# zju3dv/pvnet

Hardware: NVIDIA H100
Metric: images/sec (480x640, K=9) backbone+vote (higher is better)
Workload: dtype tf32 (fp32 storage, fp32 accumulate; vote fp32/fp64)

## Files before the change

pvnet_b200/csrc/conv_col.cu:

```cuda
#include "conv_tc.cuh"
#include "ptx.cuh"

#include <cstdlib>
#include <mutex>
#include <new>

namespace pvnet {

int g_conv_mode = 0;

namespace {

constexpr int COL_TH = 16, COL_TW = 8;
constexpr int COL_THREADS = 384;
constexpr int HEAD_MAX = 64;

__host__ __device__ constexpr int head_pitch(int hc) { return hc <= 8 ? 8 : (hc <= 24 ? 24 : 40); }
constexpr int HEAD_CPITCH = COL_TH * COL_TW + 4;
__host__ __device__ constexpr int head_stage_floats(int hc)
{
    return COL_TH * COL_TW * head_pitch(hc) > hc * HEAD_CPITCH ? COL_TH * COL_TW * head_pitch(hc) : hc * HEAD_CPITCH;
}
__host__ __device__ constexpr int head_stage_bytes(int hc) { return (head_stage_floats(hc) * 4 + COL_TH * COL_TW + 127) & ~127; }

struct ColGeom {
    int Ho, Wo, tiles_x, tiles_y, total_tiles;
    int cin_chunks, cin_pad;
    int split_chunk;
    int pad_l, pad_t;
    int stages;
    int resident;
    int out_cs, out_co, res_cs, res_co;
    int act, round_out;
    int head_cout, head_seg, mask_esz;
    int head_nhwc;
};

__device__ __forceinline__ void head_store_tile(const ColGeom &g, uint32_t sv, uint32_t sm, float *head_out, void *mask,
                                                int img, int y0, int x0, int tid, int nthr)
{
    const int hc = g.head_cout, pp = head_pitch(hc);
    const int nx = min(COL_TW, g.Wo - x0), ny = min(COL_TH, g.Ho - y0);
    const size_t npix = (size_t)g.Ho * g.Wo;
    const bool vec = (reinterpret_cast<uintptr_t>(head_out) & 15) == 0 && (g.head_nhwc ? hc % 4 == 0 : g.Wo % 4 == 0);
    for (int u = tid; u < 32 * hc; u += nthr) {
        if (g.head_nhwc) {
            const int r = u / (2 * hc), e0 = 4 * (u - r * 2 * hc);
            if (r >= ny) continue;
            float *dst = head_out + (((size_t)img * g.Ho + y0 + r) * g.Wo + x0) * hc + e0;
            if (vec) {
                const int col = e0 / hc;
                if (col < nx)
                    *reinterpret_cast<float4 *>(dst) = ptx::lds128(sv + 4u * (uint32_t)((r * COL_TW + col) * pp + e0 - col * hc));
            } else {
#pragma unroll
                for (int i = 0; i < 4; ++i) {
                    const int col = (e0 + i) / hc;
                    if (col < nx) dst[i] = ptx::lds32(sv + 4u * (uint32_t)((r * COL_TW + col) * pp + e0 + i - col * hc));
                }
            }
        } else {
            const int co = u >> 5, r = (u >> 1) & 15, xo = 4 * (u & 1);
            if (r >= ny) continue;
            float *dst = head_out + ((size_t)img * hc + co) * npix + (size_t)(y0 + r) * g.Wo + x0 + xo;
            const uint32_t src = sv + 4u * (uint32_t)(co * HEAD_CPITCH + r * COL_TW + xo);
            if (vec) {
                if (xo < nx) *reinterpret_cast<float4 *>(dst) = ptx::lds128(src);
            } else {
#pragma unroll
                for (int i = 0; i < 4; ++i)
                    if (xo + i < nx) dst[i] = ptx::lds32(src + 4u * i);
            }
        }
    }
    if (!mask) return;
    for (int p = tid; p < COL_TH * COL_TW; p += nthr) {
        const int r = p / COL_TW, c = p % COL_TW;
        if (r >= ny || c >= nx) continue;
        const size_t pix = ((size_t)img * g.Ho + y0 + r) * g.Wo + x0 + c;
        const uint32_t v = ptx::lds8(sm + (uint32_t)p);
        if (g.mask_esz == 8) reinterpret_cast<long long *>(mask)[pix] = v;
        else reinterpret_cast<unsigned char *>(mask)[pix] = (unsigned char)v;
    }
}

template <int KC, bool HEAD, int KH, int BN, bool WIDE = false>
__global__ void __launch_bounds__(COL_THREADS, 1)
    k_conv_col(const __grid_constant__ CUtensorMap tmA, const __grid_constant__ CUtensorMap tmA2,
               const __grid_constant__ CUtensorMap tmB, const __grid_constant__ CUtensorMap tmBw, const __grid_constant__ ColGeom g,
               const float *__restrict__ bias, const float *__restrict__ res, float *__restrict__ out,
               const float *__restrict__ head_w, const float *__restrict__ head_b, float *__restrict__ head_out,
               void *__restrict__ mask)
{
    static_assert(!HEAD || BN == 32, "fused head: 32 input channels");
    static_assert(!HEAD || KC == 8, "fused head: convraw.0's 8-channel chunks");
    static_assert((KC == 16) == (KH == 4), "16-channel chunks are the 4x4 stem's, and only its");
    static_assert(!WIDE || (HEAD && KC == 8 && KH == 3), "wide first source: convraw.0 form only");
    constexpr int ROWB = KC * 4;
    constexpr int B_TILE = BN * ROWB;
    constexpr int PITCH = COL_TW + KH - 1;
    constexpr int A_BOX = (COL_TH + KH - 1) * PITCH * ROWB;
    constexpr int A_BYTES = (A_BOX + 1023) & ~1023;
    constexpr int WIDE_BOX = (COL_TH + KH - 1) * PITCH * 128;
    constexpr int WIDE_BYTES = (WIDE_BOX + 1023) & ~1023;
    extern __shared__ uint8_t smem_raw[];
    uint8_t *smem = reinterpret_cast<uint8_t *>((reinterpret_cast<uintptr_t>(smem_raw) + 1023) & ~uintptr_t(1023));
    const int n_btiles = KH * KH * g.cin_chunks;
    const int n_loads = WIDE ? 2 : g.cin_chunks;
    const int stage_bytes = WIDE ? WIDE_BYTES : A_BYTES + (g.resident ? 0 : KH * KH * B_TILE);
    uint8_t *sB = smem;
    uint8_t *sA = smem + (g.resident ? (size_t)n_btiles * B_TILE : 0);
    uint8_t *sH = sA + (size_t)g.stages * stage_bytes;
    uint8_t *sHS = sH + (HEAD ? 4096 : 0);
    const int hs_bytes = HEAD ? head_stage_bytes(g.head_cout) : 0;
    uint64_t *wfull = reinterpret_cast<uint64_t *>(sHS + 2 * hs_bytes);
    uint64_t *full = wfull + 1;
    uint64_t *empty = full + g.stages;
    uint64_t *hstaged = empty + g.stages;
    uint64_t *hfree = hstaged + 2;
    float *s_bias = reinterpret_cast<float *>(empty + g.stages + (HEAD ? 4 : 0));
    float *s_head = s_bias + 64;
    constexpr int STORE_THREADS = 96;

    const int warp = threadIdx.x >> 5, lane = threadIdx.x & 31;
    if (threadIdx.x == 0) {
        ptx::mbar_init(wfull, 1);
        for (int s = 0; s < g.stages; ++s) {
            ptx::mbar_init(&full[s], 1);
            ptx::mbar_init(&empty[s], 8);
        }
        if (HEAD)
            for (int b = 0; b < 2; ++b) {
                ptx::mbar_init(&hstaged[b], 256);
                ptx::mbar_init(&hfree[b], STORE_THREADS);
            }
        ptx::fence_barrier_init();
    }
    for (int i = threadIdx.x; i < BN; i += blockDim.x) s_bias[i] = bias[i];
    if (HEAD) {
        for (int i = threadIdx.x; i < 32; i += blockDim.x) s_head[i] = i < g.head_cout ? head_b[i] : 0.f;
        for (int i = threadIdx.x; i < 32 * 32; i += blockDim.x) {
            const int n = i >> 5, p = i & 31, q = p & 7;
            const int k = (p & ~7) + (q < 4 ? 2 * q : 2 * (q - 4) + 1);
            const float v = n < g.head_cout ? head_w[n * 32 + k] : 0.f;
            *reinterpret_cast<float *>(sH + ptx::swizzle_off((uint32_t)(n * 128 + p * 4), 128)) = v;
        }
        ptx::fence_proxy_async();
    }
    __syncthreads();
    const int tiles_per_img = g.tiles_x * g.tiles_y;

    if (warp >= 8) {
        const int pw = warp - 8;
        if (pw == 0 && lane == 0 && g.resident) {
            ptx::mbar_arrive_expect_tx(wfull, (uint32_t)(n_btiles * B_TILE));
            for (int cc = WIDE ? g.split_chunk : 0; cc < g.cin_chunks; ++cc)
                for (int t = 0; t < KH * KH; ++t)
                    ptx::tma_load_2d(sB + (size_t)(cc * KH * KH + t) * B_TILE, &tmB, wfull, t * g.cin_pad + cc * KC, 0);
            if (WIDE)
                for (int t = 0; t < KH * KH; ++t) ptx::tma_load_2d(sB + (size_t)t * BN * 128, &tmBw, wfull, t * g.cin_pad, 0);
        }
        if (HEAD && pw != 0) {
            const int tid = threadIdx.x - 9 * 32;
            int it = 0;
            for (int tile = blockIdx.x; tile < g.total_tiles; tile += gridDim.x, ++it) {
                const int b = it & 1;
                const int img = tile / tiles_per_img;
                const int trem = tile - img * tiles_per_img;
                const int tyi = trem / g.tiles_x, txi = trem - tyi * g.tiles_x;
                const uint32_t buf = ptx::smem_u32(sHS) + (uint32_t)(b * hs_bytes);
                ptx::mbar_wait(&hstaged[b], (uint32_t)(it >> 1) & 1u);
                head_store_tile(g, buf, buf + 4u * (uint32_t)head_stage_floats(g.head_cout), head_out, mask, img, tyi * COL_TH,
                                txi * COL_TW, tid, STORE_THREADS);
                ptx::mbar_arrive(&hfree[b]);
            }
            return;
        }
        if (pw != 0) return;
        int s = 0;
        uint32_t ph = 0;
        const uint32_t tx_bytes = (uint32_t)(A_BOX + (g.resident ? 0 : KH * KH * B_TILE));
        for (int tile = blockIdx.x; tile < g.total_tiles; tile += gridDim.x) {
            const int img = tile / tiles_per_img;
            const int trem = tile - img * tiles_per_img;
            const int tyi = trem / g.tiles_x, txi = trem - tyi * g.tiles_x;
            const int y0 = tyi * COL_TH, x0 = txi * COL_TW;
            for (int cc = 0; cc < n_loads; ++cc) {
                uint8_t *st = sA + (size_t)s * stage_bytes;
                if (WIDE) {
                    if (pw == 0 && lane == 0) {
                        ptx::mbar_wait(&empty[s], ph ^ 1u);
                        ptx::mbar_arrive_expect_tx(&full[s], (uint32_t)(cc == 0 ? WIDE_BOX : A_BOX));
                        ptx::tma_load_4d(st, cc == 0 ? &tmA : &tmA2, &full[s], 0, x0 - g.pad_l, y0 - g.pad_t, img);
                    }
                    __syncwarp();
                } else if (pw == 0) {
                    if (lane == 0) {
                        ptx::mbar_wait(&empty[s], ph ^ 1u);
                        ptx::mbar_arrive_expect_tx(&full[s], tx_bytes);
                        if (cc < g.split_chunk)
                            ptx::tma_load_4d(st, &tmA, &full[s], cc * KC, x0 - g.pad_l, y0 - g.pad_t, img);
                        else
                            ptx::tma_load_4d(st, &tmA2, &full[s], (cc - g.split_chunk) * KC, x0 - g.pad_l, y0 - g.pad_t, img);
                        if (!g.resident)
                            for (int t = 0; t < KH * KH; ++t)
                                ptx::tma_load_2d(st + A_BYTES + (size_t)t * B_TILE, &tmB, &full[s], t * g.cin_pad + cc * KC, 0);
                    }
                    __syncwarp();
                }
                if (++s == g.stages) {
                    s = 0;
                    ph ^= 1u;
                }
            }
        }
        return;
    }

    const int wg = warp >> 2, wq = warp & 3;
    const int g8 = lane >> 2, t4 = lane & 3;
    const uint32_t sA_u = ptx::smem_u32(sA), sB_u = ptx::smem_u32(sB);
    if (g.resident) ptx::mbar_wait(wfull, 0);
    int s = 0;
    uint32_t ph = 0;
    int it = 0;
    for (int tile = blockIdx.x; tile < g.total_tiles; tile += gridDim.x, ++it) {
        float acc[BN / 2];
#pragma unroll
        for (int i = 0; i < BN / 2; ++i) acc[i] = 0.f;
        int prev = -1;
        for (int cc = 0; cc < n_loads; ++cc) {
            ptx::mbar_wait(&full[s], ph);
            const uint32_t a0 = sA_u + (uint32_t)s * (uint32_t)stage_bytes;
            ptx::wgmma_fence();
            if (WIDE && cc == 0) {
                const uint64_t ad0 = ptx::make_kmajor_desc(a0 + (uint32_t)(8 * wg * PITCH * 128), 128, PITCH * 128);
                const uint64_t bd0 = ptx::make_kmajor_desc(sB_u, 128);
#pragma unroll
                for (int ks = 0; ks < 4; ++ks)
#pragma unroll
                    for (int t = 0; t < KH * KH; ++t)
                        ptx::Wgmma<BN>::ss(acc, ad0 + (uint64_t)(((t / KH) * PITCH + t % KH) * 128 / 16 + 2 * ks),
                                           bd0 + (uint64_t)(t * (BN * 128) / 16 + 2 * ks), (t | ks) != 0 ? 1u : 0u);
            } else {
                const int c8 = WIDE ? g.split_chunk : cc;
                const uint32_t b0 = g.resident ? sB_u + (uint32_t)(c8 * KH * KH * B_TILE) : a0 + (uint32_t)A_BYTES;
                const uint64_t ad0 = ptx::make_kmajor_desc(a0 + (uint32_t)(8 * wg * PITCH * ROWB), ROWB, PITCH * ROWB);
                const uint64_t bd0 = ptx::make_kmajor_desc(b0, ROWB);
#pragma unroll
                for (int t = 0; t < KH * KH; ++t) {
                    const uint64_t ad = ad0 + (uint64_t)(((t / KH) * PITCH + t % KH) * ROWB / 16);
                    const uint64_t bd = bd0 + (uint64_t)(t * B_TILE / 16);
#pragma unroll
                    for (int ks = 0; ks < KC / 8; ++ks)
                        ptx::Wgmma<BN>::ss(acc, ad + (uint64_t)(2 * ks), bd + (uint64_t)(2 * ks), (c8 | t | ks) != 0 ? 1u : 0u);
                }
            }
            ptx::wgmma_commit();
            ptx::wgmma_wait<1>();
            ptx::fence_regs(acc);
            if (prev >= 0 && lane == 0) ptx::mbar_arrive(&empty[prev]);
            prev = s;
            if (++s == g.stages) {
                s = 0;
                ph ^= 1u;
            }
        }
        ptx::wgmma_wait<0>();
        ptx::fence_regs(acc);
        if (lane == 0) ptx::mbar_arrive(&empty[prev]);

        const int img = tile / tiles_per_img;
        const int trem = tile - img * tiles_per_img;
        const int tyi = trem / g.tiles_x, txi = trem - tyi * g.tiles_x;
        const int ty = 8 * wg + 2 * wq;
        if constexpr (!HEAD) {
            bool ok[2];
            size_t pix[2];
#pragma unroll
            for (int h = 0; h < 2; ++h) {
                const int y = tyi * COL_TH + ty + h, x = txi * COL_TW + g8;
                ok[h] = y < g.Ho && x < g.Wo;
                pix[h] = ok[h] ? ((size_t)img * g.Ho + y) * g.Wo + x : 0;
            }
            float2 rv[2][BN / 8];
            if (res) {
#pragma unroll
                for (int h = 0; h < 2; ++h)
#pragma unroll
                    for (int j = 0; j < BN / 8; ++j)
                        rv[h][j] = ok[h] ? __ldg(reinterpret_cast<const float2 *>(res + pix[h] * g.res_cs + g.res_co + 8 * j + 2 * t4))
                                         : make_float2(0.f, 0.f);
            }
#pragma unroll
            for (int h = 0; h < 2; ++h) {
                if (!ok[h]) continue;
                float *optr = out + pix[h] * g.out_cs + g.out_co;
#pragma unroll
                for (int j = 0; j < BN / 8; ++j) {
                    const int c = 8 * j + 2 * t4;
                    float2 v = make_float2(acc[4 * j + 2 * h] + s_bias[c], acc[4 * j + 2 * h + 1] + s_bias[c + 1]);
                    if (res) {
                        v.x += rv[h][j].x;
                        v.y += rv[h][j].y;
                    }
                    v.x = epi_act(v.x, g.act, g.round_out);
                    v.y = epi_act(v.y, g.act, g.round_out);
                    *reinterpret_cast<float2 *>(optr + c) = v;
                }
            }
        } else {
            uint32_t a2[4][4];
#pragma unroll
            for (int j = 0; j < 4; ++j)
#pragma unroll
                for (int f = 0; f < 4; ++f) {
                    const int r = 4 * j + ((f & 1) << 1) + (f >> 1);
                    const int c = 8 * j + 2 * t4 + (f >> 1);
                    a2[j][f] = __float_as_uint(ptx::round_tf32(epi_act(acc[r] + s_bias[c], g.act, g.round_out)));
                }
            float hacc[16];
#pragma unroll
            for (int i = 0; i < 16; ++i) hacc[i] = 0.f;
            const uint64_t hd = ptx::make_kmajor_desc(ptx::smem_u32(sH), 128);
            ptx::wgmma_fence();
#pragma unroll
            for (int j = 0; j < 4; ++j) ptx::Wgmma<32>::rs(hacc, a2[j], hd + (uint64_t)(2 * j), j != 0 ? 1u : 0u);
            ptx::wgmma_commit();
            ptx::wgmma_wait<0>();
            ptx::fence_regs(hacc);
            const int hc = g.head_cout, pp = head_pitch(hc);
            const uint32_t sv = ptx::smem_u32(sHS) + (uint32_t)((it & 1) * hs_bytes);
            const uint32_t sm = sv + 4u * (uint32_t)head_stage_floats(hc);
            ptx::mbar_wait(&hfree[it & 1], ((uint32_t)(it >> 1) & 1u) ^ 1u);
#pragma unroll
            for (int h = 0; h < 2; ++h) {
                const uint32_t p = (uint32_t)((ty + h) * COL_TW + g8);
                float best = -INFINITY;
                int best_c = 0;
#pragma unroll
                for (int j = 0; j < 4; ++j) {
                    const int co = 8 * j + 2 * t4;
                    float val[2];
#pragma unroll
                    for (int e = 0; e < 2; ++e) {
                        val[e] = hacc[4 * j + 2 * h + e] + s_head[co + e];
                        if (co + e < g.head_seg && val[e] > best) {
                            best = val[e];
                            best_c = co + e;
                        }
                    }
                    if (co < hc) {
                        if (g.head_nhwc) {
                            ptx::sts64(sv + 4u * (p * pp + co), make_float2(val[0], val[1]));
                        } else {
                            ptx::sts32(sv + 4u * (co * HEAD_CPITCH + p), val[0]);
                            if (co + 1 < hc) ptx::sts32(sv + 4u * ((co + 1) * HEAD_CPITCH + p), val[1]);
                        }
                    }
                }
#pragma unroll
                for (int o = 1; o < 4; o <<= 1) {
                    const float ob = __shfl_xor_sync(0xffffffffu, best, o);
                    const int oc = __shfl_xor_sync(0xffffffffu, best_c, o);
                    if (ob > best || (ob == best && oc < best_c)) {
                        best = ob;
                        best_c = oc;
                    }
                }
                if (t4 == 0) ptx::sts8(sm + p, (uint32_t)best_c);
            }
            ptx::mbar_arrive(&hstaged[it & 1]);
        }
    }
}

struct ColPlan {
    CUtensorMap tmA, tmA2, tmB, tmBw;
    ColGeom g;
    int kc, ksize, head, bn, wide;
    unsigned grid;
    size_t smem;
    const float *bias, *res;
    float *out;
    HeadDesc hd;
};

constexpr size_t SMEM_LIMIT = 227 * 1024;

int col_kc(int Cin) { return Cin % 32 == 0 ? 32 : (Cin == 16 ? 16 : 8); }
int col_cin_pad(int Cin) { return Cin == 16 ? 16 : (Cin + 31) / 32 * 32; }

size_t col_smem(int kc, int ksize, int cin_chunks, int bn, int stages, bool head, bool resident)
{
    const size_t rowb = (size_t)kc * 4;
    const size_t a_box = (size_t)(COL_TH + ksize - 1) * (COL_TW + ksize - 1) * rowb;
    const size_t a = (a_box + 1023) & ~(size_t)1023, bt = (size_t)bn * rowb;
    return 1024 + (resident ? (size_t)ksize * ksize * cin_chunks * bt : 0) +
           (size_t)stages * (a + (resident ? 0 : (size_t)ksize * ksize * bt)) + (head ? 4096 : 0) +
           (size_t)(1 + 2 * stages) * 8 + (64 + 32) * 4;
}

template <int KC, bool HEAD, int KH, int BN, bool WIDE = false>
int col_launch(const ColPlan &p, cudaStream_t s)
{
    if (p.bn != BN || p.kc != KC || p.ksize != KH || p.head != (HEAD ? 1 : 0) || p.wide != (WIDE ? 1 : 0)) {
        set_error("conv(col): no kernel instantiation for this plan (Cout %d, chunk %d, ksize %d)", p.bn, p.kc, p.ksize);
        return PVNET_E_STATE;
    }
    auto fn = k_conv_col<KC, HEAD, KH, BN, WIDE>;
    const cudaError_t attr_err = ensure_max_smem((const void *)fn, (int)SMEM_LIMIT);
    PV_CUDA(attr_err);
    const HeadDesc &h = p.hd;
    fn<<<p.grid, COL_THREADS, p.smem, s>>>(p.tmA, p.tmA2, p.tmB, p.tmBw, p.g, p.bias, p.res, p.out, p.head ? h.w : nullptr,
                                           p.head ? h.bias : nullptr, p.head ? h.out_nchw : nullptr,
                                           p.head ? h.mask : nullptr);
    PV_LAUNCHED("k_conv_col");
    return PVNET_OK;
}

}

bool conv_col_eligible(const ConvDesc &d)
{
    if ((d.ksize != 3 && d.ksize != 4) || d.stride != 1 || d.dilation != 1 || d.Cout > 64 || d.Cout % 32 != 0)
        return false;
    const int cin = d.Cin + d.Cin2;
    const int kc = col_kc(cin);
    if (d.Cin % kc != 0 || d.Cin2 % kc != 0) return false;
    if ((d.ksize == 4) != (kc == 16)) return false;
    return col_smem(kc, d.ksize, (cin + kc - 1) / kc, d.Cout, 2, true, false) <= SMEM_LIMIT;
}

size_t conv_col_plan_size() { return sizeof(ColPlan); }

int conv_col_plan_at(const ConvDesc &d, const HeadDesc *head, void *storage)
{
    ColPlan *p = new (storage) ColPlan();
    PV_CHECK_ARG(conv_col_eligible(d), "conv(col): layer not eligible for the column kernel");
    PV_CHECK_ARG(d.in && d.w && d.bias && (d.out || head), "conv(col): null pointer");
    PV_CHECK_ARG(d.in_cs % 4 == 0 && d.in_co % 4 == 0 && d.out_cs % 4 == 0 && d.out_co % 4 == 0,
                 "conv(col): channel strides/offsets must be multiples of 4 floats");
    PV_CHECK_ARG(!d.res || (d.res_cs % 4 == 0 && d.res_co % 4 == 0), "conv(col): residual stride/offset alignment");
    PV_CHECK_ARG(!head || (d.Cout == 32 && col_kc(d.Cin + d.Cin2) == 8 && head->cout >= 1 && head->cout <= 32 && head->w && head->bias &&
                           head->out_nchw && (!head->mask || head->mask_esz == 1 || head->mask_esz == 8)),
                 "conv(col): bad fused-head description");
    const int kc = col_kc(d.Cin + d.Cin2);
    ColGeom &g = p->g;
    g.pad_l = g.pad_t = d.ksize == 4 ? 2 : 1;
    g.Ho = d.H;
    g.Wo = d.W;
    g.tiles_x = (d.W + COL_TW - 1) / COL_TW;
    g.tiles_y = (d.H + COL_TH - 1) / COL_TH;
    g.total_tiles = g.tiles_x * g.tiles_y * d.b;
    g.cin_chunks = (d.Cin + d.Cin2) / kc;
    g.split_chunk = d.in2 ? d.Cin / kc : g.cin_chunks;
    g.cin_pad = col_cin_pad(d.Cin + d.Cin2);
    g.out_cs = d.out_cs;
    g.out_co = d.out_co;
    g.res_cs = d.res_cs;
    g.res_co = d.res_co;
    g.act = d.act;
    g.round_out = d.round_out;
    g.head_cout = head ? head->cout : 0;
    g.head_seg = head ? head->seg_dim : 0;
    g.mask_esz = head ? head->mask_esz : 0;
    g.head_nhwc = 0;
    const bool hd = head != nullptr;
    const size_t hs = hd ? 2 * (size_t)head_stage_bytes(head->cout) + 4 * 8 : 0;
    bool wide = hd && d.in2 && d.Cin == 32 && d.Cin2 == 8 && kc == 8 && d.ksize == 3;
    const size_t wx = col_smem(32, 3, 0, 0, 1, false, false) - col_smem(8, 3, 0, 0, 1, false, false);
    int stages = 8;
    bool resident = true;
    while (stages > 2 && col_smem(kc, d.ksize, g.cin_chunks, d.Cout, stages, hd, true) + hs + (wide ? stages * wx : 0) > SMEM_LIMIT)
        --stages;
    if (col_smem(kc, d.ksize, g.cin_chunks, d.Cout, stages, hd, true) + hs + (wide ? stages * wx : 0) > SMEM_LIMIT) {
        wide = false;
        resident = false;
        stages = 8;
        while (stages > 2 && col_smem(kc, d.ksize, g.cin_chunks, d.Cout, stages, hd, false) + hs > SMEM_LIMIT) --stages;
    }
    g.stages = stages;
    g.resident = resident ? 1 : 0;
    p->smem = col_smem(kc, d.ksize, g.cin_chunks, d.Cout, stages, hd, resident) + hs + (wide ? stages * wx : 0);
    p->wide = wide ? 1 : 0;
    PV_CHECK_ARG(p->smem <= SMEM_LIMIT, "conv(col): layer does not fit in shared memory");
    p->kc = kc;
    p->ksize = d.ksize;
    p->bn = d.Cout;
    p->head = hd ? 1 : 0;
    if (head) p->hd = *head;
    {
        const float *base = d.in + d.in_co;
        cuuint64_t dims[4] = {(cuuint64_t)d.Cin, (cuuint64_t)d.W, (cuuint64_t)d.H, (cuuint64_t)d.b};
        cuuint64_t strides[3] = {(cuuint64_t)d.in_cs * 4, (cuuint64_t)d.W * d.in_cs * 4,
                                 (cuuint64_t)d.H * d.W * d.in_cs * 4};
        const int akc = wide ? 32 : kc;
        cuuint32_t box[4] = {(cuuint32_t)akc, (cuuint32_t)(COL_TW + d.ksize - 1), (cuuint32_t)(COL_TH + d.ksize - 1), 1};
        int rc = tma_encode(&p->tmA, base, 4, dims, strides, box, akc * 4);
        if (rc) return rc;
        p->tmA2 = p->tmA;
    }
    if (d.in2) {
        PV_CHECK_ARG(d.in2_cs % 4 == 0 && d.in2_co % 4 == 0 && d.Cin2 > 0, "conv(col): second source stride/offset alignment");
        cuuint64_t dims[4] = {(cuuint64_t)d.Cin2, (cuuint64_t)d.W, (cuuint64_t)d.H, (cuuint64_t)d.b};
        cuuint64_t strides[3] = {(cuuint64_t)d.in2_cs * 4, (cuuint64_t)d.W * d.in2_cs * 4,
                                 (cuuint64_t)d.H * d.W * d.in2_cs * 4};
        cuuint32_t box[4] = {(cuuint32_t)kc, (cuuint32_t)(COL_TW + d.ksize - 1), (cuuint32_t)(COL_TH + d.ksize - 1), 1};
        int rc = tma_encode(&p->tmA2, d.in2 + d.in2_co, 4, dims, strides, box, kc * 4);
        if (rc) return rc;
    }
    {
        cuuint64_t dims[2] = {(cuuint64_t)d.ksize * d.ksize * g.cin_pad, (cuuint64_t)d.Cout};
        cuuint64_t strides[1] = {(cuuint64_t)d.ksize * d.ksize * g.cin_pad * 4};
        cuuint32_t box[2] = {(cuuint32_t)kc, (cuuint32_t)d.Cout};
        int rc = tma_encode(&p->tmB, d.w, 2, dims, strides, box, kc * 4);
        if (rc) return rc;
        p->tmBw = p->tmB;
        if (wide) {
            box[0] = 32;
            if ((rc = tma_encode(&p->tmBw, d.w, 2, dims, strides, box, 128))) return rc;
        }
    }
    PV_CHECK_ARG(!head || (uintptr_t)head->w % 16 == 0, "conv(col): head weights must be 16-byte aligned");
    long long grid = (long long)sm_count();
    if (grid > g.total_tiles) grid = g.total_tiles;
    p->grid = (unsigned)grid;
    p->bias = d.bias;
    p->res = d.res;
    p->out = d.out;
    return PVNET_OK;
}

void conv_col_set_head_ptrs(void *storage, float *out_nchw, void *mask, int mask_esz, int nhwc)
{
    ColPlan *p = static_cast<ColPlan *>(storage);
    p->g.head_nhwc = nhwc;
    p->hd.out_nchw = out_nchw;
    p->hd.mask = mask;
    p->hd.mask_esz = mask_esz;
    p->g.mask_esz = mask_esz;
}

int conv_col_launch_at(const void *storage, cudaStream_t s)
{
    const ColPlan &p = *static_cast<const ColPlan *>(storage);
    if (p.wide) return col_launch<8, true, 3, 32, true>(p, s);
    if (p.head) return col_launch<8, true, 3, 32>(p, s);
    const bool n64 = p.bn == 64;
    if (p.ksize == 4) return n64 ? col_launch<16, false, 4, 64>(p, s) : col_launch<16, false, 4, 32>(p, s);
    if (p.kc == 32) return n64 ? col_launch<32, false, 3, 64>(p, s) : col_launch<32, false, 3, 32>(p, s);
    return n64 ? col_launch<8, false, 3, 64>(p, s) : col_launch<8, false, 3, 32>(p, s);
}

}

extern "C" {
int pvnet_conv_set_mode(int mode)
{
    PV_CHECK_ARG(mode >= 0 && mode <= 2, "mode must be 0, 1 or 2");
    pvnet::g_conv_mode = mode;
    return PVNET_OK;
}
}
```

pvnet_b200/csrc/ptx.cuh:

```cuda
#pragma once
#include <cstdint>
#include <cuda.h>
#include <cuda_runtime.h>

namespace ptx {

__device__ __forceinline__ uint32_t smem_u32(const void *p)
{
    return static_cast<uint32_t>(__cvta_generic_to_shared(p));
}

__device__ __forceinline__ bool elect_one()
{
    uint32_t pred = 0;
    asm volatile(
        "{\n\t"
        ".reg .pred P1;\n\t"
        "elect.sync _|P1, 0xffffffff;\n\t"
        "selp.b32 %0, 1, 0, P1;\n\t"
        "}\n"
        : "=r"(pred));
    return pred != 0;
}

__device__ __forceinline__ void mbar_init(uint64_t *bar, uint32_t count)
{
    asm volatile("mbarrier.init.shared::cta.b64 [%0], %1;" ::"r"(smem_u32(bar)), "r"(count));
}
__device__ __forceinline__ void fence_barrier_init()
{
    asm volatile("fence.mbarrier_init.release.cluster;" ::: "memory");
}
__device__ __forceinline__ void fence_proxy_async()
{
    asm volatile("fence.proxy.async.shared::cta;" ::: "memory");
}
__device__ __forceinline__ void mbar_arrive_expect_tx(uint64_t *bar, uint32_t bytes)
{
    asm volatile("mbarrier.arrive.expect_tx.shared::cta.b64 _, [%0], %1;" ::"r"(smem_u32(bar)), "r"(bytes)
                 : "memory");
}
__device__ __forceinline__ void mbar_arrive(uint64_t *bar)
{
    asm volatile("mbarrier.arrive.shared::cta.b64 _, [%0];" ::"r"(smem_u32(bar)) : "memory");
}
__device__ __forceinline__ bool mbar_try_wait(uint64_t *bar, uint32_t parity)
{
    uint32_t ok;
    asm volatile(
        "{\n\t"
        ".reg .pred P1;\n\t"
        "mbarrier.try_wait.parity.shared::cta.b64 P1, [%1], %2;\n\t"
        "selp.b32 %0, 1, 0, P1;\n\t"
        "}\n"
        : "=r"(ok)
        : "r"(smem_u32(bar)), "r"(parity)
        : "memory");
    return ok != 0;
}
__device__ __forceinline__ bool mbar_test_wait(uint64_t *bar, uint32_t parity)
{
    uint32_t ok;
    asm volatile(
        "{\n\t"
        ".reg .pred P1;\n\t"
        "mbarrier.test_wait.parity.shared::cta.b64 P1, [%1], %2;\n\t"
        "selp.b32 %0, 1, 0, P1;\n\t"
        "}\n"
        : "=r"(ok)
        : "r"(smem_u32(bar)), "r"(parity)
        : "memory");
    return ok != 0;
}
__device__ __forceinline__ void mbar_wait(uint64_t *bar, uint32_t parity)
{
    while (!mbar_try_wait(bar, parity)) {
    }
}

__device__ __forceinline__ void prefetch_tensormap(const CUtensorMap *m)
{
    asm volatile("prefetch.tensormap [%0];" ::"l"(reinterpret_cast<uint64_t>(m)) : "memory");
}
__device__ __forceinline__ void tma_load_4d(void *smem_dst, const CUtensorMap *m, uint64_t *bar, int c0, int c1,
                                            int c2, int c3)
{
    asm volatile(
        "cp.async.bulk.tensor.4d.shared::cluster.global.mbarrier::complete_tx::bytes [%0], [%1, {%3, %4, %5, %6}], [%2];"
        ::"r"(smem_u32(smem_dst)), "l"(reinterpret_cast<uint64_t>(m)), "r"(smem_u32(bar)), "r"(c0), "r"(c1), "r"(c2),
        "r"(c3)
        : "memory");
}
__device__ __forceinline__ void tma_load_2d(void *smem_dst, const CUtensorMap *m, uint64_t *bar, int c0, int c1)
{
    asm volatile(
        "cp.async.bulk.tensor.2d.shared::cluster.global.mbarrier::complete_tx::bytes [%0], [%1, {%3, %4}], [%2];"
        ::"r"(smem_u32(smem_dst)), "l"(reinterpret_cast<uint64_t>(m)), "r"(smem_u32(bar)), "r"(c0), "r"(c1)
        : "memory");
}

__device__ __forceinline__ void tma_store_4d(const CUtensorMap *m, const void *smem_src, int c0, int c1, int c2, int c3)
{
    asm volatile("cp.async.bulk.tensor.4d.global.shared::cta.bulk_group [%0, {%2, %3, %4, %5}], [%1];" ::"l"(
                     reinterpret_cast<uint64_t>(m)),
                 "r"(smem_u32(smem_src)), "r"(c0), "r"(c1), "r"(c2), "r"(c3)
                 : "memory");
}
__device__ __forceinline__ void tma_store_commit() { asm volatile("cp.async.bulk.commit_group;" ::: "memory"); }
__device__ __forceinline__ void tma_store_wait_read() { asm volatile("cp.async.bulk.wait_group.read 0;" ::: "memory"); }
__device__ __forceinline__ void tma_store_wait_read1() { asm volatile("cp.async.bulk.wait_group.read 1;" ::: "memory"); }
__device__ __forceinline__ void tma_store_wait_all() { asm volatile("cp.async.bulk.wait_group 0;" ::: "memory"); }
__device__ __forceinline__ void sts128(uint32_t addr, float4 v)
{
    asm volatile("st.shared.v4.f32 [%0], {%1, %2, %3, %4};" ::"r"(addr), "f"(v.x), "f"(v.y), "f"(v.z), "f"(v.w) : "memory");
}
__device__ __forceinline__ float4 lds128(uint32_t addr)
{
    float4 v;
    asm volatile("ld.shared.v4.f32 {%0, %1, %2, %3}, [%4];" : "=f"(v.x), "=f"(v.y), "=f"(v.z), "=f"(v.w) : "r"(addr) : "memory");
    return v;
}
__device__ __forceinline__ void sts64(uint32_t addr, float2 v)
{
    asm volatile("st.shared.v2.f32 [%0], {%1, %2};" ::"r"(addr), "f"(v.x), "f"(v.y) : "memory");
}
__device__ __forceinline__ float2 lds64(uint32_t addr)
{
    float2 v;
    asm volatile("ld.shared.v2.f32 {%0, %1}, [%2];" : "=f"(v.x), "=f"(v.y) : "r"(addr) : "memory");
    return v;
}
__device__ __forceinline__ void sts32(uint32_t addr, float v) { asm volatile("st.shared.f32 [%0], %1;" ::"r"(addr), "f"(v) : "memory"); }
__device__ __forceinline__ float lds32(uint32_t addr)
{
    float v;
    asm volatile("ld.shared.f32 %0, [%1];" : "=f"(v) : "r"(addr) : "memory");
    return v;
}
__device__ __forceinline__ void sts8(uint32_t addr, uint32_t v) { asm volatile("st.shared.u8 [%0], %1;" ::"r"(addr), "r"(v) : "memory"); }
__device__ __forceinline__ uint32_t lds8(uint32_t addr)
{
    uint32_t v;
    asm volatile("ld.shared.u8 %0, [%1];" : "=r"(v) : "r"(addr) : "memory");
    return v;
}
__device__ __forceinline__ void tma_store_4d_u32(const CUtensorMap *m, uint32_t smem_src, int c0, int c1, int c2, int c3)
{
    asm volatile("cp.async.bulk.tensor.4d.global.shared::cta.bulk_group [%0, {%2, %3, %4, %5}], [%1];" ::"l"(
                     reinterpret_cast<uint64_t>(m)),
                 "r"(smem_src), "r"(c0), "r"(c1), "r"(c2), "r"(c3)
                 : "memory");
}
__device__ __forceinline__ void named_bar_sync(int id, int nthreads)
{
    asm volatile("bar.sync %0, %1;" ::"r"(id), "r"(nthreads) : "memory");
}

__device__ __forceinline__ uint32_t cluster_ctarank()
{
    uint32_t r;
    asm volatile("mov.u32 %0, %%cluster_ctarank;" : "=r"(r));
    return r;
}
__device__ __forceinline__ void cluster_sync()
{
    asm volatile("barrier.cluster.arrive.release.aligned;\n\tbarrier.cluster.wait.acquire.aligned;" ::: "memory");
}
__device__ __forceinline__ uint32_t mapa(const void *p, uint32_t rank)
{
    uint32_t r;
    asm volatile("mapa.shared::cluster.u32 %0, %1, %2;" : "=r"(r) : "r"(smem_u32(p)), "r"(rank));
    return r;
}
__device__ __forceinline__ float ld_cluster_f32(uint32_t addr)
{
    float v;
    asm volatile("ld.shared::cluster.f32 %0, [%1];" : "=f"(v) : "r"(addr) : "memory");
    return v;
}
__device__ __forceinline__ unsigned long long ld_cluster_u64(uint32_t addr)
{
    unsigned long long v;
    asm volatile("ld.shared::cluster.u64 %0, [%1];" : "=l"(v) : "r"(addr) : "memory");
    return v;
}

__device__ __forceinline__ void wgmma_fence() { asm volatile("wgmma.fence.sync.aligned;" ::: "memory"); }
__device__ __forceinline__ void wgmma_commit() { asm volatile("wgmma.commit_group.sync.aligned;" ::: "memory"); }
template <int N>
__device__ __forceinline__ void wgmma_wait() { asm volatile("wgmma.wait_group.sync.aligned %0;" ::"n"(N) : "memory"); }
template <int R>
__device__ __forceinline__ void fence_regs(float (&d)[R])
{
#pragma unroll
    for (int i = 0; i < R; ++i) asm volatile("" : "+f"(d[i])::"memory");
}

template <int N>
struct Wgmma;
template <>
struct Wgmma<32> {
    __device__ __forceinline__ static void ss(float (&d)[16], uint64_t adesc, uint64_t bdesc, uint32_t accumulate)
    {
        asm volatile(
            "{\n\t.reg .pred p;\n\tsetp.ne.b32 p, %18, 0;\n\t"
            "wgmma.mma_async.sync.aligned.m64n32k8.f32.tf32.tf32 {%0, %1, %2, %3, %4, %5, %6, %7, %8, %9, %10, %11, %12, %13, %14, %15}, %16, %17, p, 1, 1;\n\t}\n"
            : "+f"(d[0]), "+f"(d[1]), "+f"(d[2]), "+f"(d[3]), "+f"(d[4]), "+f"(d[5]), "+f"(d[6]), "+f"(d[7]), "+f"(d[8]), "+f"(d[9]), "+f"(d[10]), "+f"(d[11]), "+f"(d[12]), "+f"(d[13]), "+f"(d[14]), "+f"(d[15])
            : "l"(adesc), "l"(bdesc), "r"(accumulate));
    }
    __device__ __forceinline__ static void rs(float (&d)[16], const uint32_t (&a)[4], uint64_t bdesc, uint32_t accumulate)
    {
        asm volatile(
            "{\n\t.reg .pred p;\n\tsetp.ne.b32 p, %21, 0;\n\t"
            "wgmma.mma_async.sync.aligned.m64n32k8.f32.tf32.tf32 {%0, %1, %2, %3, %4, %5, %6, %7, %8, %9, %10, %11, %12, %13, %14, %15}, {%16, %17, %18, %19}, %20, p, 1, 1;\n\t}\n"
            : "+f"(d[0]), "+f"(d[1]), "+f"(d[2]), "+f"(d[3]), "+f"(d[4]), "+f"(d[5]), "+f"(d[6]), "+f"(d[7]), "+f"(d[8]), "+f"(d[9]), "+f"(d[10]), "+f"(d[11]), "+f"(d[12]), "+f"(d[13]), "+f"(d[14]), "+f"(d[15])
            : "r"(a[0]), "r"(a[1]), "r"(a[2]), "r"(a[3]), "l"(bdesc), "r"(accumulate));
    }
};

template <>
struct Wgmma<64> {
    __device__ __forceinline__ static void ss(float (&d)[32], uint64_t adesc, uint64_t bdesc, uint32_t accumulate)
    {
        asm volatile(
            "{\n\t.reg .pred p;\n\tsetp.ne.b32 p, %34, 0;\n\t"
            "wgmma.mma_async.sync.aligned.m64n64k8.f32.tf32.tf32 {%0, %1, %2, %3, %4, %5, %6, %7, %8, %9, %10, %11, %12, %13, %14, %15, %16, %17, %18, %19, %20, %21, %22, %23, %24, %25, %26, %27, %28, %29, %30, %31}, %32, %33, p, 1, 1;\n\t}\n"
            : "+f"(d[0]), "+f"(d[1]), "+f"(d[2]), "+f"(d[3]), "+f"(d[4]), "+f"(d[5]), "+f"(d[6]), "+f"(d[7]), "+f"(d[8]), "+f"(d[9]), "+f"(d[10]), "+f"(d[11]), "+f"(d[12]), "+f"(d[13]), "+f"(d[14]), "+f"(d[15]), "+f"(d[16]), "+f"(d[17]), "+f"(d[18]), "+f"(d[19]), "+f"(d[20]), "+f"(d[21]), "+f"(d[22]), "+f"(d[23]), "+f"(d[24]), "+f"(d[25]), "+f"(d[26]), "+f"(d[27]), "+f"(d[28]), "+f"(d[29]), "+f"(d[30]), "+f"(d[31])
            : "l"(adesc), "l"(bdesc), "r"(accumulate));
    }
    __device__ __forceinline__ static void rs(float (&d)[32], const uint32_t (&a)[4], uint64_t bdesc, uint32_t accumulate)
    {
        asm volatile(
            "{\n\t.reg .pred p;\n\tsetp.ne.b32 p, %37, 0;\n\t"
            "wgmma.mma_async.sync.aligned.m64n64k8.f32.tf32.tf32 {%0, %1, %2, %3, %4, %5, %6, %7, %8, %9, %10, %11, %12, %13, %14, %15, %16, %17, %18, %19, %20, %21, %22, %23, %24, %25, %26, %27, %28, %29, %30, %31}, {%32, %33, %34, %35}, %36, p, 1, 1;\n\t}\n"
            : "+f"(d[0]), "+f"(d[1]), "+f"(d[2]), "+f"(d[3]), "+f"(d[4]), "+f"(d[5]), "+f"(d[6]), "+f"(d[7]), "+f"(d[8]), "+f"(d[9]), "+f"(d[10]), "+f"(d[11]), "+f"(d[12]), "+f"(d[13]), "+f"(d[14]), "+f"(d[15]), "+f"(d[16]), "+f"(d[17]), "+f"(d[18]), "+f"(d[19]), "+f"(d[20]), "+f"(d[21]), "+f"(d[22]), "+f"(d[23]), "+f"(d[24]), "+f"(d[25]), "+f"(d[26]), "+f"(d[27]), "+f"(d[28]), "+f"(d[29]), "+f"(d[30]), "+f"(d[31])
            : "r"(a[0]), "r"(a[1]), "r"(a[2]), "r"(a[3]), "l"(bdesc), "r"(accumulate));
    }
};

template <>
struct Wgmma<128> {
    __device__ __forceinline__ static void ss(float (&d)[64], uint64_t adesc, uint64_t bdesc, uint32_t accumulate)
    {
        asm volatile(
            "{\n\t.reg .pred p;\n\tsetp.ne.b32 p, %66, 0;\n\t"
            "wgmma.mma_async.sync.aligned.m64n128k8.f32.tf32.tf32 {%0, %1, %2, %3, %4, %5, %6, %7, %8, %9, %10, %11, %12, %13, %14, %15, %16, %17, %18, %19, %20, %21, %22, %23, %24, %25, %26, %27, %28, %29, %30, %31, %32, %33, %34, %35, %36, %37, %38, %39, %40, %41, %42, %43, %44, %45, %46, %47, %48, %49, %50, %51, %52, %53, %54, %55, %56, %57, %58, %59, %60, %61, %62, %63}, %64, %65, p, 1, 1;\n\t}\n"
            : "+f"(d[0]), "+f"(d[1]), "+f"(d[2]), "+f"(d[3]), "+f"(d[4]), "+f"(d[5]), "+f"(d[6]), "+f"(d[7]), "+f"(d[8]), "+f"(d[9]), "+f"(d[10]), "+f"(d[11]), "+f"(d[12]), "+f"(d[13]), "+f"(d[14]), "+f"(d[15]), "+f"(d[16]), "+f"(d[17]), "+f"(d[18]), "+f"(d[19]), "+f"(d[20]), "+f"(d[21]), "+f"(d[22]), "+f"(d[23]), "+f"(d[24]), "+f"(d[25]), "+f"(d[26]), "+f"(d[27]), "+f"(d[28]), "+f"(d[29]), "+f"(d[30]), "+f"(d[31]), "+f"(d[32]), "+f"(d[33]), "+f"(d[34]), "+f"(d[35]), "+f"(d[36]), "+f"(d[37]), "+f"(d[38]), "+f"(d[39]), "+f"(d[40]), "+f"(d[41]), "+f"(d[42]), "+f"(d[43]), "+f"(d[44]), "+f"(d[45]), "+f"(d[46]), "+f"(d[47]), "+f"(d[48]), "+f"(d[49]), "+f"(d[50]), "+f"(d[51]), "+f"(d[52]), "+f"(d[53]), "+f"(d[54]), "+f"(d[55]), "+f"(d[56]), "+f"(d[57]), "+f"(d[58]), "+f"(d[59]), "+f"(d[60]), "+f"(d[61]), "+f"(d[62]), "+f"(d[63])
            : "l"(adesc), "l"(bdesc), "r"(accumulate));
    }
    __device__ __forceinline__ static void rs(float (&d)[64], const uint32_t (&a)[4], uint64_t bdesc, uint32_t accumulate)
    {
        asm volatile(
            "{\n\t.reg .pred p;\n\tsetp.ne.b32 p, %69, 0;\n\t"
            "wgmma.mma_async.sync.aligned.m64n128k8.f32.tf32.tf32 {%0, %1, %2, %3, %4, %5, %6, %7, %8, %9, %10, %11, %12, %13, %14, %15, %16, %17, %18, %19, %20, %21, %22, %23, %24, %25, %26, %27, %28, %29, %30, %31, %32, %33, %34, %35, %36, %37, %38, %39, %40, %41, %42, %43, %44, %45, %46, %47, %48, %49, %50, %51, %52, %53, %54, %55, %56, %57, %58, %59, %60, %61, %62, %63}, {%64, %65, %66, %67}, %68, p, 1, 1;\n\t}\n"
            : "+f"(d[0]), "+f"(d[1]), "+f"(d[2]), "+f"(d[3]), "+f"(d[4]), "+f"(d[5]), "+f"(d[6]), "+f"(d[7]), "+f"(d[8]), "+f"(d[9]), "+f"(d[10]), "+f"(d[11]), "+f"(d[12]), "+f"(d[13]), "+f"(d[14]), "+f"(d[15]), "+f"(d[16]), "+f"(d[17]), "+f"(d[18]), "+f"(d[19]), "+f"(d[20]), "+f"(d[21]), "+f"(d[22]), "+f"(d[23]), "+f"(d[24]), "+f"(d[25]), "+f"(d[26]), "+f"(d[27]), "+f"(d[28]), "+f"(d[29]), "+f"(d[30]), "+f"(d[31]), "+f"(d[32]), "+f"(d[33]), "+f"(d[34]), "+f"(d[35]), "+f"(d[36]), "+f"(d[37]), "+f"(d[38]), "+f"(d[39]), "+f"(d[40]), "+f"(d[41]), "+f"(d[42]), "+f"(d[43]), "+f"(d[44]), "+f"(d[45]), "+f"(d[46]), "+f"(d[47]), "+f"(d[48]), "+f"(d[49]), "+f"(d[50]), "+f"(d[51]), "+f"(d[52]), "+f"(d[53]), "+f"(d[54]), "+f"(d[55]), "+f"(d[56]), "+f"(d[57]), "+f"(d[58]), "+f"(d[59]), "+f"(d[60]), "+f"(d[61]), "+f"(d[62]), "+f"(d[63])
            : "r"(a[0]), "r"(a[1]), "r"(a[2]), "r"(a[3]), "l"(bdesc), "r"(accumulate));
    }
};

template <>
struct Wgmma<256> {
    __device__ __forceinline__ static void ss(float (&d)[128], uint64_t adesc, uint64_t bdesc, uint32_t accumulate)
    {
        asm volatile(
            "{\n\t.reg .pred p;\n\tsetp.ne.b32 p, %130, 0;\n\t"
            "wgmma.mma_async.sync.aligned.m64n256k8.f32.tf32.tf32 {%0, %1, %2, %3, %4, %5, %6, %7, %8, %9, %10, %11, %12, %13, %14, %15, %16, %17, %18, %19, %20, %21, %22, %23, %24, %25, %26, %27, %28, %29, %30, %31, %32, %33, %34, %35, %36, %37, %38, %39, %40, %41, %42, %43, %44, %45, %46, %47, %48, %49, %50, %51, %52, %53, %54, %55, %56, %57, %58, %59, %60, %61, %62, %63, %64, %65, %66, %67, %68, %69, %70, %71, %72, %73, %74, %75, %76, %77, %78, %79, %80, %81, %82, %83, %84, %85, %86, %87, %88, %89, %90, %91, %92, %93, %94, %95, %96, %97, %98, %99, %100, %101, %102, %103, %104, %105, %106, %107, %108, %109, %110, %111, %112, %113, %114, %115, %116, %117, %118, %119, %120, %121, %122, %123, %124, %125, %126, %127}, %128, %129, p, 1, 1;\n\t}\n"
            : "+f"(d[0]), "+f"(d[1]), "+f"(d[2]), "+f"(d[3]), "+f"(d[4]), "+f"(d[5]), "+f"(d[6]), "+f"(d[7]), "+f"(d[8]), "+f"(d[9]), "+f"(d[10]), "+f"(d[11]), "+f"(d[12]), "+f"(d[13]), "+f"(d[14]), "+f"(d[15]), "+f"(d[16]), "+f"(d[17]), "+f"(d[18]), "+f"(d[19]), "+f"(d[20]), "+f"(d[21]), "+f"(d[22]), "+f"(d[23]), "+f"(d[24]), "+f"(d[25]), "+f"(d[26]), "+f"(d[27]), "+f"(d[28]), "+f"(d[29]), "+f"(d[30]), "+f"(d[31]), "+f"(d[32]), "+f"(d[33]), "+f"(d[34]), "+f"(d[35]), "+f"(d[36]), "+f"(d[37]), "+f"(d[38]), "+f"(d[39]), "+f"(d[40]), "+f"(d[41]), "+f"(d[42]), "+f"(d[43]), "+f"(d[44]), "+f"(d[45]), "+f"(d[46]), "+f"(d[47]), "+f"(d[48]), "+f"(d[49]), "+f"(d[50]), "+f"(d[51]), "+f"(d[52]), "+f"(d[53]), "+f"(d[54]), "+f"(d[55]), "+f"(d[56]), "+f"(d[57]), "+f"(d[58]), "+f"(d[59]), "+f"(d[60]), "+f"(d[61]), "+f"(d[62]), "+f"(d[63]), "+f"(d[64]), "+f"(d[65]), "+f"(d[66]), "+f"(d[67]), "+f"(d[68]), "+f"(d[69]), "+f"(d[70]), "+f"(d[71]), "+f"(d[72]), "+f"(d[73]), "+f"(d[74]), "+f"(d[75]), "+f"(d[76]), "+f"(d[77]), "+f"(d[78]), "+f"(d[79]), "+f"(d[80]), "+f"(d[81]), "+f"(d[82]), "+f"(d[83]), "+f"(d[84]), "+f"(d[85]), "+f"(d[86]), "+f"(d[87]), "+f"(d[88]), "+f"(d[89]), "+f"(d[90]), "+f"(d[91]), "+f"(d[92]), "+f"(d[93]), "+f"(d[94]), "+f"(d[95]), "+f"(d[96]), "+f"(d[97]), "+f"(d[98]), "+f"(d[99]), "+f"(d[100]), "+f"(d[101]), "+f"(d[102]), "+f"(d[103]), "+f"(d[104]), "+f"(d[105]), "+f"(d[106]), "+f"(d[107]), "+f"(d[108]), "+f"(d[109]), "+f"(d[110]), "+f"(d[111]), "+f"(d[112]), "+f"(d[113]), "+f"(d[114]), "+f"(d[115]), "+f"(d[116]), "+f"(d[117]), "+f"(d[118]), "+f"(d[119]), "+f"(d[120]), "+f"(d[121]), "+f"(d[122]), "+f"(d[123]), "+f"(d[124]), "+f"(d[125]), "+f"(d[126]), "+f"(d[127])
            : "l"(adesc), "l"(bdesc), "r"(accumulate));
    }
};

__device__ __forceinline__ float round_tf32(float x)
{
    uint32_t r;
    asm("cvt.rna.tf32.f32 %0, %1;" : "=r"(r) : "f"(x));
    return __uint_as_float(r);
}


__device__ __forceinline__ uint64_t make_kmajor_desc(uint32_t smem_addr, uint32_t swizzle_bytes)
{
    const uint64_t layout = swizzle_bytes == 128 ? 1ull : (swizzle_bytes == 64 ? 2ull : 3ull);
    const uint64_t sbo = (8ull * swizzle_bytes) >> 4;
    return (uint64_t)((smem_addr & 0x3ffff) >> 4) | (1ull << 16) | (sbo << 32) | (layout << 62);
}
__device__ __forceinline__ uint64_t make_kmajor_desc(uint32_t smem_addr, uint32_t swizzle_bytes, uint32_t sbo_bytes)
{
    const uint64_t layout = swizzle_bytes == 128 ? 1ull : (swizzle_bytes == 64 ? 2ull : 3ull);
    return (uint64_t)((smem_addr & 0x3ffff) >> 4) | (1ull << 16) | ((uint64_t)(sbo_bytes >> 4) << 32) | (layout << 62);
}
__device__ __forceinline__ uint32_t swizzle_off(uint32_t off, uint32_t swizzle_bytes)
{
    return off ^ ((off >> 3) & (swizzle_bytes - 16u));
}

}
```

Baseline: 1727.

## Transpose 3x3 Cout-64 conv GEMM so pixels form N, with taller streamed tiles

For 3x3 convolutions with 64 output channels, the kernel now swaps GEMM operands: the weights become the M=64 side and a tile's pixels become the N side (128, or 192 with a new 24-row tile), so each warpgroup owns a whole tile and the two warpgroups alternate tiles using separate full barriers. When weights are streamed rather than resident and chunks are 32 channels wide, the planner picks taller 24-row tiles to reuse each streamed weight tile over more pixels. The epilogue is rewritten for the transposed accumulator layout, which uses scalar strided stores instead of float2 stores and needs more per-thread accumulator registers.

```diff
diff --git a/pvnet_b200/csrc/conv_col.cu b/pvnet_b200/csrc/conv_col.cu
--- a/pvnet_b200/csrc/conv_col.cu
+++ b/pvnet_b200/csrc/conv_col.cu
@@ -12,8 +12,11 @@
 namespace {
 
 constexpr int COL_TH = 16, COL_TW = 8;
+constexpr int COL_TH_STREAMED = 24;
 constexpr int COL_THREADS = 384;
 constexpr int HEAD_MAX = 64;
+
+__host__ __device__ constexpr bool col_transposed(int ksize, int bn) { return bn == 64 && ksize == 3; }
 
 __host__ __device__ constexpr int head_pitch(int hc) { return hc <= 8 ? 8 : (hc <= 24 ? 24 : 40); }
 constexpr int HEAD_CPITCH = COL_TH * COL_TW + 4;
@@ -84,7 +87,7 @@
     }
 }
 
-template <int KC, bool HEAD, int KH, int BN, bool WIDE = false>
+template <int KC, bool HEAD, int KH, int BN, bool WIDE = false, int TH = COL_TH>
 __global__ void __launch_bounds__(COL_THREADS, 1)
     k_conv_col(const __grid_constant__ CUtensorMap tmA, const __grid_constant__ CUtensorMap tmA2,
                const __grid_constant__ CUtensorMap tmB, const __grid_constant__ CUtensorMap tmBw, const __grid_constant__ ColGeom g,
@@ -96,10 +99,14 @@
     static_assert(!HEAD || KC == 8, "fused head: convraw.0's 8-channel chunks");
     static_assert((KC == 16) == (KH == 4), "16-channel chunks are the 4x4 stem's, and only its");
     static_assert(!WIDE || (HEAD && KC == 8 && KH == 3), "wide first source: convraw.0 form only");
+    constexpr bool TR = col_transposed(KH, BN);
+    static_assert(!TR || !HEAD, "fused head: pixel-M form only");
+    static_assert(TH == COL_TH || (TR && KC == 32), "taller tiles: transposed form with 32-channel chunks only");
+    constexpr int NPIX = TH * COL_TW;
     constexpr int ROWB = KC * 4;
     constexpr int B_TILE = BN * ROWB;
     constexpr int PITCH = COL_TW + KH - 1;
-    constexpr int A_BOX = (COL_TH + KH - 1) * PITCH * ROWB;
+    constexpr int A_BOX = (TH + KH - 1) * PITCH * ROWB;
     constexpr int A_BYTES = (A_BOX + 1023) & ~1023;
     constexpr int WIDE_BOX = (COL_TH + KH - 1) * PITCH * 128;
     constexpr int WIDE_BYTES = (WIDE_BOX + 1023) & ~1023;
@@ -115,7 +122,7 @@
     const int hs_bytes = HEAD ? head_stage_bytes(g.head_cout) : 0;
     uint64_t *wfull = reinterpret_cast<uint64_t *>(sHS + 2 * hs_bytes);
     uint64_t *full = wfull + 1;
-    uint64_t *empty = full + g.stages;
+    uint64_t *empty = full + (TR ? 2 : 1) * g.stages;
     uint64_t *hstaged = empty + g.stages;
     uint64_t *hfree = hstaged + 2;
     float *s_bias = reinterpret_cast<float *>(empty + g.stages + (HEAD ? 4 : 0));
@@ -125,10 +132,8 @@
     const int warp = threadIdx.x >> 5, lane = threadIdx.x & 31;
     if (threadIdx.x == 0) {
         ptx::mbar_init(wfull, 1);
-        for (int s = 0; s < g.stages; ++s) {
-            ptx::mbar_init(&full[s], 1);
-            ptx::mbar_init(&empty[s], 8);
-        }
+        for (int s = 0; s < (TR ? 2 : 1) * g.stages; ++s) ptx::mbar_init(&full[s], 1);
+        for (int s = 0; s < g.stages; ++s) ptx::mbar_init(&empty[s], TR ? 4 : 8);
         if (HEAD)
             for (int b = 0; b < 2; ++b) {
                 ptx::mbar_init(&hstaged[b], 256);
@@ -180,31 +185,33 @@
         int s = 0;
         uint32_t ph = 0;
         const uint32_t tx_bytes = (uint32_t)(A_BOX + (g.resident ? 0 : KH * KH * B_TILE));
-        for (int tile = blockIdx.x; tile < g.total_tiles; tile += gridDim.x) {
+        int it = 0;
+        for (int tile = blockIdx.x; tile < g.total_tiles; tile += gridDim.x, ++it) {
             const int img = tile / tiles_per_img;
             const int trem = tile - img * tiles_per_img;
             const int tyi = trem / g.tiles_x, txi = trem - tyi * g.tiles_x;
-            const int y0 = tyi * COL_TH, x0 = txi * COL_TW;
+            const int y0 = tyi * TH, x0 = txi * COL_TW;
+            uint64_t *fb = full + (TR ? (it & 1) * g.stages : 0);
             for (int cc = 0; cc < n_loads; ++cc) {
                 uint8_t *st = sA + (size_t)s * stage_bytes;
                 if (WIDE) {
                     if (pw == 0 && lane == 0) {
                         ptx::mbar_wait(&empty[s], ph ^ 1u);
-                        ptx::mbar_arrive_expect_tx(&full[s], (uint32_t)(cc == 0 ? WIDE_BOX : A_BOX));
-                        ptx::tma_load_4d(st, cc == 0 ? &tmA : &tmA2, &full[s], 0, x0 - g.pad_l, y0 - g.pad_t, img);
+                        ptx::mbar_arrive_expect_tx(&fb[s], (uint32_t)(cc == 0 ? WIDE_BOX : A_BOX));
+                        ptx::tma_load_4d(st, cc == 0 ? &tmA : &tmA2, &fb[s], 0, x0 - g.pad_l, y0 - g.pad_t, img);
                     }
                     __syncwarp();
                 } else if (pw == 0) {
                     if (lane == 0) {
                         ptx::mbar_wait(&empty[s], ph ^ 1u);
-                        ptx::mbar_arrive_expect_tx(&full[s], tx_bytes);
+                        ptx::mbar_arrive_expect_tx(&fb[s], tx_bytes);
                         if (cc < g.split_chunk)
-                            ptx::tma_load_4d(st, &tmA, &full[s], cc * KC, x0 - g.pad_l, y0 - g.pad_t, img);
+                            ptx::tma_load_4d(st, &tmA, &fb[s], cc * KC, x0 - g.pad_l, y0 - g.pad_t, img);
                         else
-                            ptx::tma_load_4d(st, &tmA2, &full[s], (cc - g.split_chunk) * KC, x0 - g.pad_l, y0 - g.pad_t, img);
+                            ptx::tma_load_4d(st, &tmA2, &fb[s], (cc - g.split_chunk) * KC, x0 - g.pad_l, y0 - g.pad_t, img);
                         if (!g.resident)
                             for (int t = 0; t < KH * KH; ++t)
-                                ptx::tma_load_2d(st + A_BYTES + (size_t)t * B_TILE, &tmB, &full[s], t * g.cin_pad + cc * KC, 0);
+                                ptx::tma_load_2d(st + A_BYTES + (size_t)t * B_TILE, &tmB, &fb[s], t * g.cin_pad + cc * KC, 0);
                     }
                     __syncwarp();
                 }
@@ -221,156 +228,237 @@
     const int g8 = lane >> 2, t4 = lane & 3;
     const uint32_t sA_u = ptx::smem_u32(sA), sB_u = ptx::smem_u32(sB);
     if (g.resident) ptx::mbar_wait(wfull, 0);
-    int s = 0;
-    uint32_t ph = 0;
-    int it = 0;
-    for (int tile = blockIdx.x; tile < g.total_tiles; tile += gridDim.x, ++it) {
-        float acc[BN / 2];
-#pragma unroll
-        for (int i = 0; i < BN / 2; ++i) acc[i] = 0.f;
-        int prev = -1;
-        for (int cc = 0; cc < n_loads; ++cc) {
-            ptx::mbar_wait(&full[s], ph);
-            const uint32_t a0 = sA_u + (uint32_t)s * (uint32_t)stage_bytes;
-            ptx::wgmma_fence();
-            if (WIDE && cc == 0) {
-                const uint64_t ad0 = ptx::make_kmajor_desc(a0 + (uint32_t)(8 * wg * PITCH * 128), 128, PITCH * 128);
-                const uint64_t bd0 = ptx::make_kmajor_desc(sB_u, 128);
-#pragma unroll
-                for (int ks = 0; ks < 4; ++ks)
-#pragma unroll
-                    for (int t = 0; t < KH * KH; ++t)
-                        ptx::Wgmma<BN>::ss(acc, ad0 + (uint64_t)(((t / KH) * PITCH + t % KH) * 128 / 16 + 2 * ks),
-                                           bd0 + (uint64_t)(t * (BN * 128) / 16 + 2 * ks), (t | ks) != 0 ? 1u : 0u);
+
+    if constexpr (TR) {
+        const int c0 = 16 * wq + g8;
+        const float bias0 = s_bias[c0], bias1 = s_bias[c0 + 8];
+        uint64_t *fw = full + wg * g.stages;
+        uint32_t fph = 0;
+        for (int it = wg, tile = blockIdx.x + wg * gridDim.x; tile < g.total_tiles; it += 2, tile += 2 * gridDim.x) {
+            int s = it * n_loads % g.stages;
+            float acc[NPIX / 2];
+#pragma unroll
+            for (int i = 0; i < NPIX / 2; ++i) acc[i] = 0.f;
+            int prev = -1;
+            for (int cc = 0; cc < n_loads; ++cc) {
+                ptx::mbar_wait(&fw[s], (fph >> s) & 1u);
+                fph ^= 1u << s;
+                const uint32_t a0 = sA_u + (uint32_t)s * (uint32_t)stage_bytes;
+                const uint32_t b0 = g.resident ? sB_u + (uint32_t)(cc * KH * KH * B_TILE) : a0 + (uint32_t)A_BYTES;
+                const uint64_t wd0 = ptx::make_kmajor_desc(b0, ROWB);
+                const uint64_t xd0 = ptx::make_kmajor_desc(a0, ROWB, PITCH * ROWB);
+                ptx::wgmma_fence();
+#pragma unroll
+                for (int t = 0; t < KH * KH; ++t) {
+                    const uint64_t wd = wd0 + (uint64_t)(t * B_TILE / 16);
+                    const uint64_t xd = xd0 + (uint64_t)(((t / KH) * PITCH + t % KH) * ROWB / 16);
+#pragma unroll
+                    for (int ks = 0; ks < KC / 8; ++ks)
+                        ptx::Wgmma<NPIX>::ss(acc, wd + (uint64_t)(2 * ks), xd + (uint64_t)(2 * ks), (cc | t | ks) != 0 ? 1u : 0u);
+                }
+                ptx::wgmma_commit();
+                ptx::wgmma_wait<1>();
+                ptx::fence_regs(acc);
+                if (prev >= 0 && lane == 0) ptx::mbar_arrive(&empty[prev]);
+                prev = s;
+                if (++s == g.stages) s = 0;
+            }
+            ptx::wgmma_wait<0>();
+            ptx::fence_regs(acc);
+            if (lane == 0) ptx::mbar_arrive(&empty[prev]);
+
+            const int img = tile / tiles_per_img;
+            const int trem = tile - img * tiles_per_img;
+            const int tyi = trem / g.tiles_x, txi = trem - tyi * g.tiles_x;
+            const int y0 = tyi * TH, x = txi * COL_TW + 2 * t4;
+            const size_t pix0 = ((size_t)img * g.Ho + y0) * g.Wo + x;
+            const bool okx[2] = {x < g.Wo, x + 1 < g.Wo};
+            const int ny = min(TH, g.Ho - y0);
+            constexpr int RB = TH % 16 == 0 ? 16 : 8;
+            const float *rp = res ? res + pix0 * g.res_cs + g.res_co + c0 : nullptr;
+            float *op = out + pix0 * g.out_cs + g.out_co + c0;
+#pragma unroll
+            for (int jb = 0; jb < TH; jb += RB) {
+                float rv[4 * RB];
+                if (res) {
+#pragma unroll
+                    for (int j = 0; j < RB; ++j)
+#pragma unroll
+                        for (int e = 0; e < 2; ++e) {
+                            const bool ok = jb + j < ny && okx[e];
+                            const float *p = rp + ((size_t)(jb + j) * g.Wo + e) * g.res_cs;
+                            rv[4 * j + e] = ok ? __ldg(p) : 0.f;
+                            rv[4 * j + 2 + e] = ok ? __ldg(p + 8) : 0.f;
+                        }
+                }
+#pragma unroll
+                for (int j = 0; j < RB; ++j)
+#pragma unroll
+                    for (int e = 0; e < 2; ++e) {
+                        if (jb + j >= ny || !okx[e]) continue;
+                        float v0 = acc[4 * (jb + j) + e] + bias0, v1 = acc[4 * (jb + j) + 2 + e] + bias1;
+                        if (res) {
+                            v0 += rv[4 * j + e];
+                            v1 += rv[4 * j + 2 + e];
+                        }
+                        float *p = op + ((size_t)(jb + j) * g.Wo + e) * g.out_cs;
+                        p[0] = epi_act(v0, g.act, g.round_out);
+                        p[8] = epi_act(v1, g.act, g.round_out);
+                    }
+            }
+        }
+    } else {
+        int s = 0;
+        uint32_t ph = 0;
+        int it = 0;
+        for (int tile = blockIdx.x; tile < g.total_tiles; tile += gridDim.x, ++it) {
+            float acc[BN / 2];
+#pragma unroll
+            for (int i = 0; i < BN / 2; ++i) acc[i] = 0.f;
+            int prev = -1;
+            for (int cc = 0; cc < n_loads; ++cc) {
+                ptx::mbar_wait(&full[s], ph);
+                const uint32_t a0 = sA_u + (uint32_t)s * (uint32_t)stage_bytes;
+                ptx::wgmma_fence();
+                if (WIDE && cc == 0) {
+                    const uint64_t ad0 = ptx::make_kmajor_desc(a0 + (uint32_t)(8 * wg * PITCH * 128), 128, PITCH * 128);
+                    const uint64_t bd0 = ptx::make_kmajor_desc(sB_u, 128);
+#pragma unroll
+                    for (int ks = 0; ks < 4; ++ks)
+#pragma unroll
+                        for (int t = 0; t < KH * KH; ++t)
+                            ptx::Wgmma<BN>::ss(acc, ad0 + (uint64_t)(((t / KH) * PITCH + t % KH) * 128 / 16 + 2 * ks),
+                                               bd0 + (uint64_t)(t * (BN * 128) / 16 + 2 * ks), (t | ks) != 0 ? 1u : 0u);
+                } else {
+                    const int c8 = WIDE ? g.split_chunk : cc;
+                    const uint32_t b0 = g.resident ? sB_u + (uint32_t)(c8 * KH * KH * B_TILE) : a0 + (uint32_t)A_BYTES;
+                    const uint64_t ad0 = ptx::make_kmajor_desc(a0 + (uint32_t)(8 * wg * PITCH * ROWB), ROWB, PITCH * ROWB);
+                    const uint64_t bd0 = ptx::make_kmajor_desc(b0, ROWB);
+#pragma unroll
+                    for (int t = 0; t < KH * KH; ++t) {
+                        const uint64_t ad = ad0 + (uint64_t)(((t / KH) * PITCH + t % KH) * ROWB / 16);
+                        const uint64_t bd = bd0 + (uint64_t)(t * B_TILE / 16);
+#pragma unroll
+                        for (int ks = 0; ks < KC / 8; ++ks)
+                            ptx::Wgmma<BN>::ss(acc, ad + (uint64_t)(2 * ks), bd + (uint64_t)(2 * ks), (c8 | t | ks) != 0 ? 1u : 0u);
+                    }
+                }
+                ptx::wgmma_commit();
+                ptx::wgmma_wait<1>();
+                ptx::fence_regs(acc);
+                if (prev >= 0 && lane == 0) ptx::mbar_arrive(&empty[prev]);
+                prev = s;
+                if (++s == g.stages) {
+                    s = 0;
+                    ph ^= 1u;
+                }
+            }
+            ptx::wgmma_wait<0>();
+            ptx::fence_regs(acc);
+            if (lane == 0) ptx::mbar_arrive(&empty[prev]);
+
+            const int img = tile / tiles_per_img;
+            const int trem = tile - img * tiles_per_img;
+            const int tyi = trem / g.tiles_x, txi = trem - tyi * g.tiles_x;
+            const int ty = 8 * wg + 2 * wq;
+            if constexpr (!HEAD) {
+                bool ok[2];
+                size_t pix[2];
+#pragma unroll
+                for (int h = 0; h < 2; ++h) {
+                    const int y = tyi * COL_TH + ty + h, x = txi * COL_TW + g8;
+                    ok[h] = y < g.Ho && x < g.Wo;
+                    pix[h] = ok[h] ? ((size_t)img * g.Ho + y) * g.Wo + x : 0;
+                }
+                float2 rv[2][BN / 8];
+                if (res) {
+#pragma unroll
+                    for (int h = 0; h < 2; ++h)
+#pragma unroll
+                        for (int j = 0; j < BN / 8; ++j)
+                            rv[h][j] = ok[h] ? __ldg(reinterpret_cast<const float2 *>(res + pix[h] * g.res_cs + g.res_co + 8 * j + 2 * t4))
+                                             : make_float2(0.f, 0.f);
+                }
+#pragma unroll
+                for (int h = 0; h < 2; ++h) {
+                    if (!ok[h]) continue;
+                    float *optr = out + pix[h] * g.out_cs + g.out_co;
+#pragma unroll
+                    for (int j = 0; j < BN / 8; ++j) {
+                        const int c = 8 * j + 2 * t4;
+                        float2 v = make_float2(acc[4 * j + 2 * h] + s_bias[c], acc[4 * j + 2 * h + 1] + s_bias[c + 1]);
+                        if (res) {
+                            v.x += rv[h][j].x;
+                            v.y += rv[h][j].y;
+                        }
+                        v.x = epi_act(v.x, g.act, g.round_out);
+                        v.y = epi_act(v.y, g.act, g.round_out);
+                        *reinterpret_cast<float2 *>(optr + c) = v;
+                    }
+                }
             } else {
-                const int c8 = WIDE ? g.split_chunk : cc;
-                const uint32_t b0 = g.resident ? sB_u + (uint32_t)(c8 * KH * KH * B_TILE) : a0 + (uint32_t)A_BYTES;
-                const uint64_t ad0 = ptx::make_kmajor_desc(a0 + (uint32_t)(8 * wg * PITCH * ROWB), ROWB, PITCH * ROWB);
-                const uint64_t bd0 = ptx::make_kmajor_desc(b0, ROWB);
-#pragma unroll
-                for (int t = 0; t < KH * KH; ++t) {
-                    const uint64_t ad = ad0 + (uint64_t)(((t / KH) * PITCH + t % KH) * ROWB / 16);
-                    const uint64_t bd = bd0 + (uint64_t)(t * B_TILE / 16);
-#pragma unroll
-                    for (int ks = 0; ks < KC / 8; ++ks)
-                        ptx::Wgmma<BN>::ss(acc, ad + (uint64_t)(2 * ks), bd + (uint64_t)(2 * ks), (c8 | t | ks) != 0 ? 1u : 0u);
-                }
-            }
-            ptx::wgmma_commit();
-            ptx::wgmma_wait<1>();
-            ptx::fence_regs(acc);
-            if (prev >= 0 && lane == 0) ptx::mbar_arrive(&empty[prev]);
-            prev = s;
-            if (++s == g.stages) {
-                s = 0;
-                ph ^= 1u;
-            }
-        }
-        ptx::wgmma_wait<0>();
-        ptx::fence_regs(acc);
-        if (lane == 0) ptx::mbar_arrive(&empty[prev]);
-
-        const int img = tile / tiles_per_img;
-        const int trem = tile - img * tiles_per_img;
-        const int tyi = trem / g.tiles_x, txi = trem - tyi * g.tiles_x;
-        const int ty = 8 * wg + 2 * wq;
-        if constexpr (!HEAD) {
-            bool ok[2];
-            size_t pix[2];
-#pragma unroll
-            for (int h = 0; h < 2; ++h) {
-                const int y = tyi * COL_TH + ty + h, x = txi * COL_TW + g8;
-                ok[h] = y < g.Ho && x < g.Wo;
-                pix[h] = ok[h] ? ((size_t)img * g.Ho + y) * g.Wo + x : 0;
-            }
-            float2 rv[2][BN / 8];
-            if (res) {
-#pragma unroll
-                for (int h = 0; h < 2; ++h)
-#pragma unroll
-                    for (int j = 0; j < BN / 8; ++j)
-                        rv[h][j] = ok[h] ? __ldg(reinterpret_cast<const float2 *>(res + pix[h] * g.res_cs + g.res_co + 8 * j + 2 * t4))
-                                         : make_float2(0.f, 0.f);
-            }
-#pragma unroll
-            for (int h = 0; h < 2; ++h) {
-                if (!ok[h]) continue;
-                float *optr = out + pix[h] * g.out_cs + g.out_co;
-#pragma unroll
-                for (int j = 0; j < BN / 8; ++j) {
-                    const int c = 8 * j + 2 * t4;
-                    float2 v = make_float2(acc[4 * j + 2 * h] + s_bias[c], acc[4 * j + 2 * h + 1] + s_bias[c + 1]);
-                    if (res) {
-                        v.x += rv[h][j].x;
-                        v.y += rv[h][j].y;
-                    }
-                    v.x = epi_act(v.x, g.act, g.round_out);
-                    v.y = epi_act(v.y, g.act, g.round_out);
-                    *reinterpret_cast<float2 *>(optr + c) = v;
-                }
-            }
-        } else {
-            uint32_t a2[4][4];
-#pragma unroll
-            for (int j = 0; j < 4; ++j)
-#pragma unroll
-                for (int f = 0; f < 4; ++f) {
-                    const int r = 4 * j + ((f & 1) << 1) + (f >> 1);
-                    const int c = 8 * j + 2 * t4 + (f >> 1);
-                    a2[j][f] = __float_as_uint(ptx::round_tf32(epi_act(acc[r] + s_bias[c], g.act, g.round_out)));
-                }
-            float hacc[16];
-#pragma unroll
-            for (int i = 0; i < 16; ++i) hacc[i] = 0.f;
-            const uint64_t hd = ptx::make_kmajor_desc(ptx::smem_u32(sH), 128);
-            ptx::wgmma_fence();
-#pragma unroll
-            for (int j = 0; j < 4; ++j) ptx::Wgmma<32>::rs(hacc, a2[j], hd + (uint64_t)(2 * j), j != 0 ? 1u : 0u);
-            ptx::wgmma_commit();
-            ptx::wgmma_wait<0>();
-            ptx::fence_regs(hacc);
-            const int hc = g.head_cout, pp = head_pitch(hc);
-            const uint32_t sv = ptx::smem_u32(sHS) + (uint32_t)((it & 1) * hs_bytes);
-            const uint32_t sm = sv + 4u * (uint32_t)head_stage_floats(hc);
-            ptx::mbar_wait(&hfree[it & 1], ((uint32_t)(it >> 1) & 1u) ^ 1u);
-#pragma unroll
-            for (int h = 0; h < 2; ++h) {
-                const uint32_t p = (uint32_t)((ty + h) * COL_TW + g8);
-                float best = -INFINITY;
-                int best_c = 0;
-#pragma unroll
-                for (int j = 0; j < 4; ++j) {
-                    const int co = 8 * j + 2 * t4;
-                    float val[2];
-#pragma unroll
-                    for (int e = 0; e < 2; ++e) {
-                        val[e] = hacc[4 * j + 2 * h + e] + s_head[co + e];
-                        if (co + e < g.head_seg && val[e] > best) {
-                            best = val[e];
-                            best_c = co + e;
+                uint32_t a2[4][4];
+#pragma unroll
+                for (int j = 0; j < 4; ++j)
+#pragma unroll
+                    for (int f = 0; f < 4; ++f) {
+                        const int r = 4 * j + ((f & 1) << 1) + (f >> 1);
+                        const int c = 8 * j + 2 * t4 + (f >> 1);
+                        a2[j][f] = __float_as_uint(ptx::round_tf32(epi_act(acc[r] + s_bias[c], g.act, g.round_out)));
+                    }
+                float hacc[16];
+#pragma unroll
+                for (int i = 0; i < 16; ++i) hacc[i] = 0.f;
+                const uint64_t hd = ptx::make_kmajor_desc(ptx::smem_u32(sH), 128);
+                ptx::wgmma_fence();
+#pragma unroll
+                for (int j = 0; j < 4; ++j) ptx::Wgmma<32>::rs(hacc, a2[j], hd + (uint64_t)(2 * j), j != 0 ? 1u : 0u);
+                ptx::wgmma_commit();
+                ptx::wgmma_wait<0>();
+                ptx::fence_regs(hacc);
+                const int hc = g.head_cout, pp = head_pitch(hc);
+                const uint32_t sv = ptx::smem_u32(sHS) + (uint32_t)((it & 1) * hs_bytes);
+                const uint32_t sm = sv + 4u * (uint32_t)head_stage_floats(hc);
+                ptx::mbar_wait(&hfree[it & 1], ((uint32_t)(it >> 1) & 1u) ^ 1u);
+#pragma unroll
+                for (int h = 0; h < 2; ++h) {
+                    const uint32_t p = (uint32_t)((ty + h) * COL_TW + g8);
+                    float best = -INFINITY;
+                    int best_c = 0;
+#pragma unroll
+                    for (int j = 0; j < 4; ++j) {
+                        const int co = 8 * j + 2 * t4;
+                        float val[2];
+#pragma unroll
+                        for (int e = 0; e < 2; ++e) {
+                            val[e] = hacc[4 * j + 2 * h + e] + s_head[co + e];
+                            if (co + e < g.head_seg && val[e] > best) {
+                                best = val[e];
+                                best_c = co + e;
+                            }
                         }
-                    }
-                    if (co < hc) {
-                        if (g.head_nhwc) {
-                            ptx::sts64(sv + 4u * (p * pp + co), make_float2(val[0], val[1]));
-                        } else {
-                            ptx::sts32(sv + 4u * (co * HEAD_CPITCH + p), val[0]);
-                            if (co + 1 < hc) ptx::sts32(sv + 4u * ((co + 1) * HEAD_CPITCH + p), val[1]);
+                        if (co < hc) {
+                            if (g.head_nhwc) {
+                                ptx::sts64(sv + 4u * (p * pp + co), make_float2(val[0], val[1]));
+                            } else {
+                                ptx::sts32(sv + 4u * (co * HEAD_CPITCH + p), val[0]);
+                                if (co + 1 < hc) ptx::sts32(sv + 4u * ((co + 1) * HEAD_CPITCH + p), val[1]);
+                            }
                         }
                     }
-                }
-#pragma unroll
-                for (int o = 1; o < 4; o <<= 1) {
-                    const float ob = __shfl_xor_sync(0xffffffffu, best, o);
-                    const int oc = __shfl_xor_sync(0xffffffffu, best_c, o);
-                    if (ob > best || (ob == best && oc < best_c)) {
-                        best = ob;
-                        best_c = oc;
-                    }
-                }
-                if (t4 == 0) ptx::sts8(sm + p, (uint32_t)best_c);
-            }
-            ptx::mbar_arrive(&hstaged[it & 1]);
+#pragma unroll
+                    for (int o = 1; o < 4; o <<= 1) {
+                        const float ob = __shfl_xor_sync(0xffffffffu, best, o);
+                        const int oc = __shfl_xor_sync(0xffffffffu, best_c, o);
+                        if (ob > best || (ob == best && oc < best_c)) {
+                            best = ob;
+                            best_c = oc;
+                        }
+                    }
+                    if (t4 == 0) ptx::sts8(sm + p, (uint32_t)best_c);
+                }
+                ptx::mbar_arrive(&hstaged[it & 1]);
+            }
         }
     }
 }
@@ -378,7 +466,7 @@
 struct ColPlan {
     CUtensorMap tmA, tmA2, tmB, tmBw;
     ColGeom g;
-    int kc, ksize, head, bn, wide;
+    int kc, ksize, head, bn, wide, th;
     unsigned grid;
     size_t smem;
     const float *bias, *res;
@@ -391,24 +479,24 @@
 int col_kc(int Cin) { return Cin % 32 == 0 ? 32 : (Cin == 16 ? 16 : 8); }
 int col_cin_pad(int Cin) { return Cin == 16 ? 16 : (Cin + 31) / 32 * 32; }
 
-size_t col_smem(int kc, int ksize, int cin_chunks, int bn, int stages, bool head, bool resident)
+size_t col_smem(int kc, int ksize, int cin_chunks, int bn, int stages, bool head, bool resident, int th = COL_TH)
 {
     const size_t rowb = (size_t)kc * 4;
-    const size_t a_box = (size_t)(COL_TH + ksize - 1) * (COL_TW + ksize - 1) * rowb;
+    const size_t a_box = (size_t)(th + ksize - 1) * (COL_TW + ksize - 1) * rowb;
     const size_t a = (a_box + 1023) & ~(size_t)1023, bt = (size_t)bn * rowb;
     return 1024 + (resident ? (size_t)ksize * ksize * cin_chunks * bt : 0) +
            (size_t)stages * (a + (resident ? 0 : (size_t)ksize * ksize * bt)) + (head ? 4096 : 0) +
-           (size_t)(1 + 2 * stages) * 8 + (64 + 32) * 4;
-}
-
-template <int KC, bool HEAD, int KH, int BN, bool WIDE = false>
+           (size_t)(1 + (col_transposed(ksize, bn) ? 3 : 2) * stages) * 8 + (64 + 32) * 4;
+}
+
+template <int KC, bool HEAD, int KH, int BN, bool WIDE = false, int TH = COL_TH>
 int col_launch(const ColPlan &p, cudaStream_t s)
 {
-    if (p.bn != BN || p.kc != KC || p.ksize != KH || p.head != (HEAD ? 1 : 0) || p.wide != (WIDE ? 1 : 0)) {
+    if (p.bn != BN || p.kc != KC || p.ksize != KH || p.head != (HEAD ? 1 : 0) || p.wide != (WIDE ? 1 : 0) || p.th != TH) {
         set_error("conv(col): no kernel instantiation for this plan (Cout %d, chunk %d, ksize %d)", p.bn, p.kc, p.ksize);
         return PVNET_E_STATE;
     }
-    auto fn = k_conv_col<KC, HEAD, KH, BN, WIDE>;
+    auto fn = k_conv_col<KC, HEAD, KH, BN, WIDE, TH>;
     const cudaError_t attr_err = ensure_max_smem((const void *)fn, (int)SMEM_LIMIT);
     PV_CUDA(attr_err);
     const HeadDesc &h = p.hd;
@@ -450,9 +538,6 @@
     g.pad_l = g.pad_t = d.ksize == 4 ? 2 : 1;
     g.Ho = d.H;
     g.Wo = d.W;
-    g.tiles_x = (d.W + COL_TW - 1) / COL_TW;
-    g.tiles_y = (d.H + COL_TH - 1) / COL_TH;
-    g.total_tiles = g.tiles_x * g.tiles_y * d.b;
     g.cin_chunks = (d.Cin + d.Cin2) / kc;
     g.split_chunk = d.in2 ? d.Cin / kc : g.cin_chunks;
     g.cin_pad = col_cin_pad(d.Cin + d.Cin2);
@@ -474,15 +559,21 @@
     bool resident = true;
     while (stages > 2 && col_smem(kc, d.ksize, g.cin_chunks, d.Cout, stages, hd, true) + hs + (wide ? stages * wx : 0) > SMEM_LIMIT)
         --stages;
+    int th = COL_TH;
     if (col_smem(kc, d.ksize, g.cin_chunks, d.Cout, stages, hd, true) + hs + (wide ? stages * wx : 0) > SMEM_LIMIT) {
         wide = false;
         resident = false;
+        if (col_transposed(d.ksize, d.Cout) && kc == 32) th = COL_TH_STREAMED;
         stages = 8;
-        while (stages > 2 && col_smem(kc, d.ksize, g.cin_chunks, d.Cout, stages, hd, false) + hs > SMEM_LIMIT) --stages;
+        while (stages > 2 && col_smem(kc, d.ksize, g.cin_chunks, d.Cout, stages, hd, false, th) + hs > SMEM_LIMIT) --stages;
     }
     g.stages = stages;
     g.resident = resident ? 1 : 0;
-    p->smem = col_smem(kc, d.ksize, g.cin_chunks, d.Cout, stages, hd, resident) + hs + (wide ? stages * wx : 0);
+    g.tiles_x = (d.W + COL_TW - 1) / COL_TW;
+    g.tiles_y = (d.H + th - 1) / th;
+    g.total_tiles = g.tiles_x * g.tiles_y * d.b;
+    p->th = th;
+    p->smem = col_smem(kc, d.ksize, g.cin_chunks, d.Cout, stages, hd, resident, th) + hs + (wide ? stages * wx : 0);
     p->wide = wide ? 1 : 0;
     PV_CHECK_ARG(p->smem <= SMEM_LIMIT, "conv(col): layer does not fit in shared memory");
     p->kc = kc;
@@ -496,7 +587,7 @@
         cuuint64_t strides[3] = {(cuuint64_t)d.in_cs * 4, (cuuint64_t)d.W * d.in_cs * 4,
                                  (cuuint64_t)d.H * d.W * d.in_cs * 4};
         const int akc = wide ? 32 : kc;
-        cuuint32_t box[4] = {(cuuint32_t)akc, (cuuint32_t)(COL_TW + d.ksize - 1), (cuuint32_t)(COL_TH + d.ksize - 1), 1};
+        cuuint32_t box[4] = {(cuuint32_t)akc, (cuuint32_t)(COL_TW + d.ksize - 1), (cuuint32_t)(th + d.ksize - 1), 1};
         int rc = tma_encode(&p->tmA, base, 4, dims, strides, box, akc * 4);
         if (rc) return rc;
         p->tmA2 = p->tmA;
@@ -506,7 +597,7 @@
         cuuint64_t dims[4] = {(cuuint64_t)d.Cin2, (cuuint64_t)d.W, (cuuint64_t)d.H, (cuuint64_t)d.b};
         cuuint64_t strides[3] = {(cuuint64_t)d.in2_cs * 4, (cuuint64_t)d.W * d.in2_cs * 4,
                                  (cuuint64_t)d.H * d.W * d.in2_cs * 4};
-        cuuint32_t box[4] = {(cuuint32_t)kc, (cuuint32_t)(COL_TW + d.ksize - 1), (cuuint32_t)(COL_TH + d.ksize - 1), 1};
+        cuuint32_t box[4] = {(cuuint32_t)kc, (cuuint32_t)(COL_TW + d.ksize - 1), (cuuint32_t)(th + d.ksize - 1), 1};
         int rc = tma_encode(&p->tmA2, d.in2 + d.in2_co, 4, dims, strides, box, kc * 4);
         if (rc) return rc;
     }
@@ -549,7 +640,10 @@
     if (p.head) return col_launch<8, true, 3, 32>(p, s);
     const bool n64 = p.bn == 64;
     if (p.ksize == 4) return n64 ? col_launch<16, false, 4, 64>(p, s) : col_launch<16, false, 4, 32>(p, s);
-    if (p.kc == 32) return n64 ? col_launch<32, false, 3, 64>(p, s) : col_launch<32, false, 3, 32>(p, s);
+    if (p.kc == 32) {
+        if (!n64) return col_launch<32, false, 3, 32>(p, s);
+        return p.th == COL_TH_STREAMED ? col_launch<32, false, 3, 64, false, COL_TH_STREAMED>(p, s) : col_launch<32, false, 3, 64>(p, s);
+    }
     return n64 ? col_launch<8, false, 3, 64>(p, s) : col_launch<8, false, 3, 32>(p, s);
 }
 
diff --git a/pvnet_b200/csrc/ptx.cuh b/pvnet_b200/csrc/ptx.cuh
--- a/pvnet_b200/csrc/ptx.cuh
+++ b/pvnet_b200/csrc/ptx.cuh
@@ -259,6 +259,18 @@
 };
 
 template <>
+struct Wgmma<192> {
+    __device__ __forceinline__ static void ss(float (&d)[96], uint64_t adesc, uint64_t bdesc, uint32_t accumulate)
+    {
+        asm volatile(
+            "{\n\t.reg .pred p;\n\tsetp.ne.b32 p, %98, 0;\n\t"
+            "wgmma.mma_async.sync.aligned.m64n192k8.f32.tf32.tf32 {%0, %1, %2, %3, %4, %5, %6, %7, %8, %9, %10, %11, %12, %13, %14, %15, %16, %17, %18, %19, %20, %21, %22, %23, %24, %25, %26, %27, %28, %29, %30, %31, %32, %33, %34, %35, %36, %37, %38, %39, %40, %41, %42, %43, %44, %45, %46, %47, %48, %49, %50, %51, %52, %53, %54, %55, %56, %57, %58, %59, %60, %61, %62, %63, %64, %65, %66, %67, %68, %69, %70, %71, %72, %73, %74, %75, %76, %77, %78, %79, %80, %81, %82, %83, %84, %85, %86, %87, %88, %89, %90, %91, %92, %93, %94, %95}, %96, %97, p, 1, 1;\n\t}\n"
+            : "+f"(d[0]), "+f"(d[1]), "+f"(d[2]), "+f"(d[3]), "+f"(d[4]), "+f"(d[5]), "+f"(d[6]), "+f"(d[7]), "+f"(d[8]), "+f"(d[9]), "+f"(d[10]), "+f"(d[11]), "+f"(d[12]), "+f"(d[13]), "+f"(d[14]), "+f"(d[15]), "+f"(d[16]), "+f"(d[17]), "+f"(d[18]), "+f"(d[19]), "+f"(d[20]), "+f"(d[21]), "+f"(d[22]), "+f"(d[23]), "+f"(d[24]), "+f"(d[25]), "+f"(d[26]), "+f"(d[27]), "+f"(d[28]), "+f"(d[29]), "+f"(d[30]), "+f"(d[31]), "+f"(d[32]), "+f"(d[33]), "+f"(d[34]), "+f"(d[35]), "+f"(d[36]), "+f"(d[37]), "+f"(d[38]), "+f"(d[39]), "+f"(d[40]), "+f"(d[41]), "+f"(d[42]), "+f"(d[43]), "+f"(d[44]), "+f"(d[45]), "+f"(d[46]), "+f"(d[47]), "+f"(d[48]), "+f"(d[49]), "+f"(d[50]), "+f"(d[51]), "+f"(d[52]), "+f"(d[53]), "+f"(d[54]), "+f"(d[55]), "+f"(d[56]), "+f"(d[57]), "+f"(d[58]), "+f"(d[59]), "+f"(d[60]), "+f"(d[61]), "+f"(d[62]), "+f"(d[63]), "+f"(d[64]), "+f"(d[65]), "+f"(d[66]), "+f"(d[67]), "+f"(d[68]), "+f"(d[69]), "+f"(d[70]), "+f"(d[71]), "+f"(d[72]), "+f"(d[73]), "+f"(d[74]), "+f"(d[75]), "+f"(d[76]), "+f"(d[77]), "+f"(d[78]), "+f"(d[79]), "+f"(d[80]), "+f"(d[81]), "+f"(d[82]), "+f"(d[83]), "+f"(d[84]), "+f"(d[85]), "+f"(d[86]), "+f"(d[87]), "+f"(d[88]), "+f"(d[89]), "+f"(d[90]), "+f"(d[91]), "+f"(d[92]), "+f"(d[93]), "+f"(d[94]), "+f"(d[95])
+            : "l"(adesc), "l"(bdesc), "r"(accumulate));
+    }
+};
+
+template <>
 struct Wgmma<256> {
     __device__ __forceinline__ static void ss(float (&d)[128], uint64_t adesc, uint64_t bdesc, uint32_t accumulate)
     {
```

Result: no change. 1733 (median of 6 runs) (+0.3%).
